# element36-io/hyperfridge-r0

Hardware: NVIDIA B200
Metric: po2=20 segments/sec (synthetic rv32im-shaped segment, W=256); camt53 proof seconds measured on a 37-segment proof (camt53.proof_seconds) (higher is better)
Workload: dtype u32 (BabyBear mod p, Montgomery)

## Files before the change

### hyperfridge-r0_b200/csrc/hfb200.cu

```cuda
#include "../../include/hfb200.h"
#include "prover.cuh"
#include "probe.cuh"
#include "verify.cuh"
#include <algorithm>
#include <atomic>
#include <condition_variable>
#include <deque>
#include <map>
#include <memory>
#include <thread>

using namespace hf;

struct hfb200_ctx {
    Prover p;
    std::vector<uint32_t> seal;
#ifndef HFB200_EMU
    cudaEvent_t marks[4] = {nullptr, nullptr, nullptr, nullptr};
#endif
};

static const char kOomMessage[] = "hfb200: out of memory while reporting an error";
static const char* dup_err(const std::string& s) {
    char* m = (char*)std::malloc(s.size() + 1);
// ... 417 lines not shown
            }
            hfb200_segment_job& j = jobs[idx];
            const auto t0 = std::chrono::steady_clock::now();
            j.attempts++;
            const char* err = nullptr;
            int injected = -1;
            {
                std::lock_guard<std::mutex> lock(pool->inject_mu);
                auto it = pool->inject.find(w);
                if (it != pool->inject.end()) { if (it->second.first == 0) { injected = it->second.second; pool->inject.erase(it); } else it->second.first--; }
            }
            if (injected == 0) err = dup_err("CUDA error cudaErrorLaunchFailure (injected by hfb200_pool_inject_fault)");
            else if (injected == 1) err = dup_err("injected non-device failure");
            if (!err && !j.code) {
                const auto it = pool->control.find(j.po2);
                if (it == pool->control.end()) err = dup_err("code is NULL and no control group was loaded for this po2 (hfb200_pool_load_control)");
                else if (!(sl.ctx->p.control_cached && sl.ctx->p.po2 == j.po2 && sl.ctx->p.control_gen == it->second.gen)) {
                    uint32_t root[8];
                    err = control_root_impl(sl.ctx, j.po2, it->second.code, root, it->second.gen);
                }
            }
            if (!err && pool->accum_fn) err = prove_job_with_accum(pool, sl.ctx, j, idx);
            else if (!err) err = hfb200_prove_segment(sl.ctx, j.po2, j.globals, j.code, j.data, j.blind_seed, j.seal_out, j.seal_cap, &j.seal_words);
            j.device = sl.device;
            j.ms = std::chrono::duration<float, std::milli>(std::chrono::steady_clock::now() - t0).count();
            bool requeue = false, retire = false;
            if (err && is_device_fault(err)) {
                pool->drop_ctx(sl);
                try { sl.ctx = pool->make_ctx(sl.device); } catch (...) { sl.ctx = nullptr; retire = true; }
                requeue = j.attempts < HFB200_POOL_MAX_ATTEMPTS;
            }
            {
                std::lock_guard<std::mutex> lock(mu);
                if (err && is_device_fault(err)) { pool->total_faults++; sl.faults++; if (!retire) pool->contexts_recreated++; }
                if (requeue) { hfb200_free_error(err); err = nullptr; pool->total_retries++; pending.push_back(idx); }
                j.error = err;
                if (retire) sl.retired = true;
                inflight--;
            }
            cv.notify_all();
            if (retire) {
                std::lock_guard<std::mutex> lock(mu);
                size_t spare = pool->slots.size();
                for (size_t k = 0; k < pool->slots.size(); k++) if (!taken[k] && !pool->slots[k].retired && pool->slots[k].ctx) { spare = k; break; }
                if (spare == pool->slots.size()) return;
                taken[spare] = 1;
                w = spare;
            }
        }
    };
    std::vector<std::thread> th;
    std::map<int, size_t> started;
    for (size_t w = 0; w < pool->slots.size(); w++) {
        const auto& sl = pool->slots[w];
        if (sl.retired || !sl.ctx) continue;
        if (started[sl.device] >= per_device_cap[sl.device]) continue;
        started[sl.device]++;
        taken[w] = 1;
        th.emplace_back(worker, w);
    }
    for (auto& t : th) t.join();
    for (size_t idx : pending) if (!jobs[idx].error) jobs[idx].error = dup_err("no healthy context left in the pool (every worker retired after CUDA errors)");
    for (size_t i = 0; i < n_jobs; i++)
        if (jobs[i].error) return dup_err(std::string("job ") + std::to_string(i) + ": " + jobs[i].error);
    API_CATCH
}

const char* hfb200_pool_load_control(hfb200_pool* pool, uint32_t po2, const uint32_t* code) {
    API_TRY
    if (!pool) throw Err("hfb200_pool_load_control: NULL pool");
    if (code) pool->control[po2] = hfb200_pool::Control{code, pool->next_gen++}; else pool->control.erase(po2);
    API_CATCH
}

const char* hfb200_pool_set_accum(hfb200_pool* pool, hfb200_accum_fn fn, void* user) {
    API_TRY
    if (!pool) throw Err("hfb200_pool_set_accum: NULL pool");
    pool->accum_fn = fn;
    pool->accum_user = fn ? user : nullptr;
    API_CATCH
}

void hfb200_pool_destroy(hfb200_pool* pool) { delete pool; }

struct DevBuf {
    Dev& d; uint32_t* p;
    DevBuf(Dev& dev, size_t words) : d(dev), p((uint32_t*)dev.alloc(words * 4)) {}
    ~DevBuf() { d.free(p); }
};

const char* hfb200_op_interpolate_ntt(hfb200_ctx* ctx, uint32_t* io, size_t count, size_t n, int zk_shift) {
    API_TRY
    if (!ctx || !io) throw Err("op_interpolate_ntt: NULL argument");
    ctx->p.bind();
    Dev& d = ctx->p.dev;
    const int lg = ilog2(n);
    if ((1ull << lg) != n || lg > 24 || count == 0) throw Err("op_interpolate_ntt: bad size");
    DevBuf b(d, count * n);
    d.h2d(b.p, io, count * n * 4);
    ctx->p.ntt.interpolate(b.p, n, b.p, n, (uint32_t)count, lg, zk_shift != 0);
    d.d2h(io, b.p, count * n * 4);
    d.sync();
    API_CATCH
}
const char* hfb200_op_expand_ntt(hfb200_ctx* ctx, uint32_t* out, const uint32_t* in, size_t count, size_t n_in, uint32_t expand_bits) {
    API_TRY
    if (!ctx || !out || !in) throw Err("op_expand_ntt: NULL argument");
    ctx->p.bind();
    Dev& d = ctx->p.dev;
    const int lg = ilog2(n_in);
    if ((1ull << lg) != n_in || lg + (int)expand_bits > 24 || (expand_bits != 0 && expand_bits != 2) || count == 0) throw Err("op_expand_ntt: bad size");
    DevBuf bi(d, count * n_in), bo(d, (count * n_in) << expand_bits);
    d.h2d(bi.p, in, count * n_in * 4);
    ctx->p.ntt.expand_evaluate(bi.p, n_in, bo.p, n_in << expand_bits, (uint32_t)count, lg, (int)expand_bits);
    d.d2h(out, bo.p, ((count * n_in) << expand_bits) * 4);
    d.sync();
    API_CATCH
}
const char* hfb200_op_lde(hfb200_ctx* ctx, uint32_t* out, const uint32_t* in, size_t count, size_t n_in) {
    API_TRY
    if (!ctx || !out || !in) throw Err("op_lde: NULL argument");
    ctx->p.bind();
    Dev& d = ctx->p.dev;
    const int lg = ilog2(n_in);
    if ((1ull << lg) != n_in || lg > 22 || count == 0) throw Err("op_lde: bad size");
    DevBuf bi(d, count * n_in), bs(d, count * n_in), bo(d, count * n_in * 4);
    d.h2d(bi.p, in, count * n_in * 4);
    ctx->p.ntt.lde(bi.p, n_in, bo.p, n_in * 4, bs.p, (uint32_t)count, lg);
    d.d2h(out, bo.p, count * n_in * 16);
    d.sync();
    API_CATCH
}
const char* hfb200_op_merkle(hfb200_ctx* ctx, const uint32_t* matrix, size_t rows, size_t cols, uint32_t* nodes_out) {
    API_TRY
    if (!ctx || !matrix || !nodes_out) throw Err("op_merkle: NULL argument");
    ctx->p.bind();
    Dev& d = ctx->p.dev;
    if ((1ull << ilog2(rows)) != rows || rows < 2 || cols == 0) throw Err("op_merkle: rows must be a power of two >= 2");
    DevBuf bm(d, rows * cols), bn(d, 2 * rows * 8);
    d.h2d(bm.p, matrix, rows * cols * 4);
    d.zero(bn.p, 8 * 4);
    ctx->p.merkle.build(bm.p, rows, (uint32_t)rows, (uint32_t)cols, bn.p);
    d.d2h(nodes_out, bn.p, 2 * rows * 8 * 4);
    d.sync();
    API_CATCH
}
const char* hfb200_op_poseidon2(hfb200_ctx* ctx, uint32_t* states, size_t n) {
    API_TRY
    if (!ctx || (!states && n)) throw Err("op_poseidon2: NULL argument");
    ctx->p.bind();
    Dev& d = ctx->p.dev;
    DevBuf b(d, n * 24);
    d.h2d(b.p, states, n * 24 * 4);
    d.launch<PermuteKernel, 128, 1>((unsigned)((n + 127) / 128), 1, 128, 0, b.p, (uint32_t)n);
    d.d2h(states, b.p, n * 24 * 4);
    d.sync();
    API_CATCH
}
const char* hfb200_op_fri_fold(hfb200_ctx* ctx, uint32_t* out, const uint32_t* in, size_t n, const uint32_t* mix4) {
    API_TRY
    if (!ctx || !out || !in || !mix4) throw Err("op_fri_fold: NULL argument");
    ctx->p.bind();
    Dev& d = ctx->p.dev;
    if (n < 16 || (n & 15)) throw Err("op_fri_fold: n must be a multiple of 16");
    DevBuf bi(d, 4 * n), bo(d, 4 * n / 16);
    d.h2d(bi.p, in, 4 * n * 4);
    FriFoldArgs fa{};
    fa.in = bi.p; fa.out = bo.p; fa.n = (uint32_t)n;
    const E4 fm = e4(mix4[0], mix4[1], mix4[2], mix4[3]);
    { E4 cur = e4_one(); for (int i = 0; i < 16; i++) { fa.mixpow[i] = cur; cur = e4_mul(cur, fm); } }
    d.launch<FriFoldKernel, 256, 1>((unsigned)((n / 16 + 255) / 256), 1, 256, 0, fa);
    d.d2h(out, bo.p, (4 * n / 16) * 4);
    d.sync();
    API_CATCH
}

const char* hfb200_bench_lde(hfb200_ctx* ctx, uint32_t po2, uint32_t count, uint32_t iters, float* ms_avg) {
    API_TRY
    if (!ctx || !ms_avg) throw Err("bench_lde: NULL argument");
    Prover& p = ctx->p;
    p.bind();
    p.layout(po2);
    if (count == 0 || count > p.cir.cd.w_data) throw Err("bench_lde: count must be in [1, w_data]");
    if (!p.have_trace) throw Err("bench_lde: call hfb200_witgen_synth first");
    const size_t N = (size_t)1 << po2;
    Timer t; t.init(p.dev.stream);
    p.ntt.lde(p.tr[GROUP_DATA], N, p.ev[GROUP_DATA], 4 * N, p.scratch, count, (int)po2);
    t.start();
    for (uint32_t i = 0; i < iters; i++) p.ntt.lde(p.tr[GROUP_DATA], N, p.ev[GROUP_DATA], 4 * N, p.scratch, count, (int)po2);
    t.stop();
    *ms_avg = t.ms() / (iters ? iters : 1);
    t.destroy();
    API_CATCH
}
const char* hfb200_bench_merkle(hfb200_ctx* ctx, uint32_t po2, uint32_t count, uint32_t iters, float* ms_avg) {
    API_TRY
    if (!ctx || !ms_avg) throw Err("bench_merkle: NULL argument");
    Prover& p = ctx->p;
    p.bind();
    p.layout(po2);
    if (count == 0 || count > p.cir.cd.w_data) throw Err("bench_merkle: count must be in [1, w_data]");
    const size_t D = (size_t)4 << po2;
    Timer t; t.init(p.dev.stream);
    p.merkle.build(p.ev[GROUP_DATA], D, (uint32_t)D, count, p.nodes[GROUP_DATA]);
    t.start();
    for (uint32_t i = 0; i < iters; i++) p.merkle.build(p.ev[GROUP_DATA], D, (uint32_t)D, count, p.nodes[GROUP_DATA]);
    t.stop();
    *ms_avg = t.ms() / (iters ? iters : 1);
    t.destroy();
    API_CATCH
}

const char* hfb200_verify_segment(const hfb200_circuit_desc* c, const hfb200_circuit_ir* ir, const uint32_t* seal, size_t seal_words,
                                  const uint32_t* code_root, uint32_t* po2_out) {
    API_TRY
    if ((c == nullptr) == (ir == nullptr)) throw Err("hfb200_verify_segment: pass exactly one of circuit / ir");
    if (!seal || !code_root) throw Err("hfb200_verify_segment: NULL seal or code_root");
    VCircuit vc;
    if (c) vc.init_builtin(c->w_code, c->w_data, c->w_accum);
    else vc.init_ir(ir->w_code, ir->w_data, ir->w_accum, ir->n_mix, reinterpret_cast<const IrTap*>(ir->taps), ir->n_taps,
                    reinterpret_cast<const IrStep*>(ir->steps), ir->n_steps, ir->ret, ir->info);
    verify_segment(vc, seal, seal_words, code_root, po2_out);
    API_CATCH
}
const char* hfb200_verify_segments(const hfb200_circuit_desc* c, const hfb200_circuit_ir* ir, const uint32_t* const* seals, const size_t* seal_words,
                                   size_t n, const uint32_t* code_roots, uint32_t* po2_out, unsigned threads, size_t* first_bad) {
    API_TRY
    if ((c == nullptr) == (ir == nullptr)) throw Err("hfb200_verify_segments: pass exactly one of circuit / ir");
    if (n && (!seals || !seal_words || !code_roots)) throw Err("hfb200_verify_segments: NULL argument");
    if (first_bad) *first_bad = n;
    VCircuit vc;
    if (c) vc.init_builtin(c->w_code, c->w_data, c->w_accum);
    else vc.init_ir(ir->w_code, ir->w_data, ir->w_accum, ir->n_mix, reinterpret_cast<const IrTap*>(ir->taps), ir->n_taps,
                    reinterpret_cast<const IrStep*>(ir->steps), ir->n_steps, ir->ret, ir->info);
    p2_host_consts();
    unsigned nt = threads ? threads : std::thread::hardware_concurrency();
    if (nt == 0) nt = 1;
    if (nt > n) nt = (unsigned)n;
    std::vector<std::string> errs(n);
    std::vector<char> bad(n, 0);
    std::atomic<size_t> next{0};
    auto work = [&]() {
        for (size_t i = next.fetch_add(1); i < n; i = next.fetch_add(1)) {
            try {
                if (!seals[i]) throw Err("NULL seal");
                uint32_t po2 = 0;
                verify_segment(vc, seals[i], seal_words[i], code_roots + 8 * i, &po2);
                if (po2_out) po2_out[i] = po2;
            } catch (const std::exception& e) { errs[i] = e.what(); bad[i] = 1; } catch (...) { errs[i] = "unknown error"; bad[i] = 1; }
        }
    };
    std::vector<std::thread> pool;
    for (unsigned t = 1; t < nt; t++) pool.emplace_back(work);
    work();
    for (auto& t : pool) t.join();
    for (size_t i = 0; i < n; i++) if (bad[i]) { if (first_bad) *first_bad = i; throw Err("segment " + std::to_string(i) + ": " + errs[i]); }
    API_CATCH
}
static Digest8 digest_bytes_impl(const uint8_t* bytes, size_t n) {
    if (n >= P) throw Err("hfb200_digest_bytes: input too long");
    std::vector<uint32_t> el;
    el.reserve(1 + (n + 2) / 3);
    el.push_back(to_mont((uint32_t)n));
    for (size_t i = 0; i < n; i += 3) {
        uint32_t v = bytes[i];
        if (i + 1 < n) v |= (uint32_t)bytes[i + 1] << 8;
        if (i + 2 < n) v |= (uint32_t)bytes[i + 2] << 16;
        el.push_back(to_mont(v));
    }
    return host_hash_elems(el.data(), el.size());
}
static Digest8 digest_pair_impl(const uint32_t* a, const uint32_t* b) {
    p2_host_consts();
    uint32_t st[24] = {0};
    for (int i = 0; i < 8; i++) { st[i] = a[i]; st[8 + i] = b[i]; }
    p2_mix(st);
    Digest8 d; for (int i = 0; i < 8; i++) d.w[i] = st[i];
    return d;
}
static void claim_check_words(const uint32_t* w, const char* what) {
    for (int i = 0; i < 8; i++) if (w[i] >= P) throw Err(std::string("claim: ") + what + " digest holds a non-canonical field element");
}
const char* hfb200_digest_bytes(const uint8_t* bytes, size_t n, uint32_t* out8) {
    API_TRY
    if ((!bytes && n) || !out8) throw Err("hfb200_digest_bytes: NULL argument");
    const Digest8 d = digest_bytes_impl(bytes, n);
    std::memcpy(out8, d.w, 32);
    API_CATCH
}
const char* hfb200_digest_pair(const uint32_t* a8, const uint32_t* b8, uint32_t* out8) {
    API_TRY
    if (!a8 || !b8 || !out8) throw Err("hfb200_digest_pair: NULL argument");
    claim_check_words(a8, "left"); claim_check_words(b8, "right");
    const Digest8 d = digest_pair_impl(a8, b8);
    std::memcpy(out8, d.w, 32);
    API_CATCH
}
const char* hfb200_claim_encode(const hfb200_claim* c, uint32_t* globals) {
    API_TRY
    if (!c || !globals) throw Err("hfb200_claim_encode: NULL argument");
    if (c->exit_code > 1) throw Err("hfb200_claim_encode: exit_code must be HFB200_EXIT_HALTED or HFB200_EXIT_SYSTEM_SPLIT");
    claim_check_words(c->pre, "pre"); claim_check_words(c->post, "post"); claim_check_words(c->output, "output");
    globals[1] = c->exit_code ? ONE : 0u;
    std::memcpy(globals + 8, c->pre, 32); std::memcpy(globals + 16, c->post, 32); std::memcpy(globals + 24, c->output, 32);
    API_CATCH
}
const char* hfb200_claim_decode(const uint32_t* seal, size_t seal_words, hfb200_claim* out) {
// ... 118 lines not shown
```

### hyperfridge-r0_b200/csrc/poseidon2.cuh

```cuda
#pragma once
#include "dev.cuh"

namespace hf {

#include "poseidon2_consts.inc"

struct P2Consts {
    uint32_t rc_first[96], rc_partial[21], rc_last[96], diag[24];
    uint32_t diag_std[24], diag_shoup[24];
};

static inline P2Consts p2_make_consts() {
    P2Consts c;
    for (int i = 0; i < 96; i++) { c.rc_first[i] = to_mont(P2_RC_FULL_FIRST[i]); c.rc_last[i] = to_mont(P2_RC_FULL_LAST[i]); }
    for (int i = 0; i < 21; i++) c.rc_partial[i] = to_mont(P2_RC_PARTIAL[i]);
    for (int i = 0; i < 24; i++) {
        c.diag[i] = to_mont(P2_M_INT_DIAG[i]);
        c.diag_std[i] = P2_M_INT_DIAG[i];
        c.diag_shoup[i] = (uint32_t)(((uint64_t)P2_M_INT_DIAG[i] << 32) / P);
    }
    return c;
}

#if !defined(HFB200_EMU)
__constant__ P2Consts g_p2c;
#define P2C_DEV g_p2c
#endif
static P2Consts g_p2c_host;
static inline const P2Consts& p2_host_consts() {
    static const bool once = (g_p2c_host = p2_make_consts(), true);
    (void)once;
    return g_p2c_host;
}

HD const P2Consts& p2c() {
#if defined(__CUDA_ARCH__)
    return P2C_DEV;
#else
    return g_p2c_host;
#endif
}

#ifndef P2_FADD_ALU
#define P2_FADD_ALU 0
#endif
HD uint32_t padd(uint32_t a, uint32_t b) {
#if defined(__CUDA_ARCH__) && P2_FADD_ALU
    const uint32_t x = __viaddmin_u32(a, b, 0xFFFFFFFFu);
    return __viaddmin_u32(x, 0u - P, x);
#else
    return fadd(a, b);
#endif
}
HD uint32_t fmul_lazy(uint32_t a, uint32_t b) {
    uint64_t o = (uint64_t)a * b;
    uint32_t m = (uint32_t)o * P_INV;
#ifdef __CUDA_ARCH__
    uint32_t mp = __umulhi(m, P);
#else
    uint32_t mp = (uint32_t)(((uint64_t)m * P) >> 32);
#endif
    return (uint32_t)(o >> 32) - mp + P;
}
HD uint32_t sbox7(uint32_t x) { uint32_t x2 = fmul(x, x), x3 = fmul(x2, x), x4 = fmul_lazy(x2, x2); return fmul(x3, x4); }
HD int32_t smul(int32_t a, int32_t b) {
    const int64_t o = (int64_t)a * b;
    const int32_t m = (int32_t)((uint32_t)o * P_INV);
#ifdef __CUDA_ARCH__
    const int32_t mp = __mulhi(m, (int32_t)P);
#else
    const int32_t mp = (int32_t)(((int64_t)m * (int64_t)P) >> 32);
#endif
    return (int32_t)(o >> 32) - mp;
}
#ifndef P2_SIGNED_SBOX
#define P2_SIGNED_SBOX 1
#endif
HD uint32_t sbox7_rc(uint32_t s, uint32_t rc) {
#if P2_SIGNED_SBOX
    const int32_t x = (int32_t)(s + rc - P);
    const int32_t x2 = smul(x, x), x3 = smul(x2, x), x4 = smul(x2, x2);
    const uint32_t r = (uint32_t)smul(x3, x4);
    return umin32(r, r + P);
#else
    return sbox7(padd(s, rc));
#endif
}
HD uint32_t fmul_const(uint32_t x, uint32_t d, uint32_t dp) {
#ifdef __CUDA_ARCH__
    const uint32_t q = __umulhi(x, dp);
#else
    const uint32_t q = (uint32_t)(((uint64_t)x * dp) >> 32);
#endif
    const uint32_t r = x * d - q * P;
    return umin32(r, r - P);
}

#ifndef P2_DEFERRED_SUM
#define P2_DEFERRED_SUM 1
#endif
HD void p2_m_ext(uint32_t* s) {
#pragma unroll
    for (int c = 0; c < 24; c += 4) {
        uint32_t a = s[c], b = s[c + 1], cc = s[c + 2], d = s[c + 3];
        uint32_t t0 = padd(a, b), t1 = padd(cc, d);
        uint32_t t2 = padd(padd(b, b), t1), t3 = padd(padd(d, d), t0);
        uint32_t t4 = padd(t1, t1); t4 = padd(padd(t4, t4), t3);
        uint32_t t5 = padd(t0, t0); t5 = padd(padd(t5, t5), t2);
        s[c] = padd(t3, t5); s[c + 1] = t5; s[c + 2] = padd(t2, t4); s[c + 3] = t4;
    }
    uint32_t sum[4];
#pragma unroll
    for (int j = 0; j < 4; j++) sum[j] = padd(padd(padd(s[j], s[4 + j]), padd(s[8 + j], s[12 + j])), padd(s[16 + j], s[20 + j]));
#pragma unroll
    for (int i = 0; i < 24; i++) s[i] = padd(s[i], sum[i & 3]);
}

HD void p2_m_int(uint32_t* s, const P2Consts& k) {
    uint32_t sum = 0;
#pragma unroll
    for (int i = 0; i < 24; i++) sum = padd(sum, s[i]);
#pragma unroll
    for (int i = 0; i < 24; i++) s[i] = padd(sum, fmul_const(s[i], k.diag_std[i], k.diag_shoup[i]));
}

HD void p2_mix(uint32_t* s) {
    const P2Consts& k = p2c();
    p2_m_ext(s);
#pragma unroll 1
    for (int r = 0; r < 4; r++) {
#pragma unroll
        for (int i = 0; i < 24; i++) s[i] = sbox7_rc(s[i], k.rc_first[r * 24 + i]);
        p2_m_ext(s);
    }
#if P2_DEFERRED_SUM
    {
        uint32_t U = s[1];
#pragma unroll
        for (int i = 2; i < 24; i++) U = padd(U, s[i]);
#pragma unroll 1
        for (int r = 0; r < 21; r++) {
            s[0] = sbox7_rc(s[0], k.rc_partial[r]);
            const uint32_t S = padd(s[0], U);
            uint32_t t[24];
#pragma unroll
            for (int i = 0; i < 24; i++) t[i] = fmul_const(s[i], k.diag_std[i], k.diag_shoup[i]);
            uint32_t T = t[1];
#pragma unroll
            for (int i = 2; i < 24; i++) T = padd(T, t[i]);
#if P2_DEFERRED_SUM == 2
            uint32_t S2 = padd(S, S), S4 = padd(S2, S2), S8 = padd(S4, S4), S16 = padd(S8, S8);
            const uint32_t S23 = fsub(padd(S16, S8), S);
#else
            const uint32_t S23 = fmul_const(S, 23u, (uint32_t)((23ull << 32) / P));
#endif
            U = padd(T, S23);
            s[0] = padd(t[0], S);
#pragma unroll
            for (int i = 1; i < 24; i++) s[i] = fadd_lazy(t[i], S);
        }
#pragma unroll
        for (int i = 1; i < 24; i++) s[i] = umin32(s[i], s[i] - P);
    }
#else
#pragma unroll 1
    for (int r = 0; r < 21; r++) {
        s[0] = sbox7_rc(s[0], k.rc_partial[r]);
        p2_m_int(s, k);
    }
#endif
#pragma unroll 1
    for (int r = 0; r < 4; r++) {
#pragma unroll
        for (int i = 0; i < 24; i++) s[i] = sbox7_rc(s[i], k.rc_last[r * 24 + i]);
        p2_m_ext(s);
    }
}

struct HashRowsKernel {
    static constexpr bool kBarrier = false;
    HD static void run(const KCtx& cx, uint32_t*, const uint32_t* matrix, uint64_t col_stride, uint32_t rows, uint32_t cols, uint32_t* nodes) {
        const uint64_t r = (uint64_t)cx.bx * cx.nt + cx.tid;
        if (r >= rows) return;
        uint32_t s[24];
#pragma unroll
        for (int i = 0; i < 24; i++) s[i] = 0;
        const uint32_t* src = matrix + r;
        uint32_t c = 0;
        for (; c + 16 <= cols; c += 16) {
#pragma unroll
            for (int i = 0; i < 16; i++) s[i] = src[(uint64_t)(c + i) * col_stride];
            p2_mix(s);
        }
        if (c < cols || cols == 0) {
#pragma unroll
            for (int i = 0; i < 16; i++) s[i] = (c + i < cols) ? src[(uint64_t)(c + i) * col_stride] : 0u;
            p2_mix(s);
        }
        uint4* dst = reinterpret_cast<uint4*>(nodes + ((uint64_t)rows + r) * 8);
        dst[0] = make_uint4(s[0], s[1], s[2], s[3]);
        dst[1] = make_uint4(s[4], s[5], s[6], s[7]);
    }
};

struct HashFoldKernel {
    static constexpr bool kBarrier = false;
    HD static void run(const KCtx& cx, uint32_t*, uint32_t* nodes, uint32_t level_size) {
        const uint64_t t = (uint64_t)cx.bx * cx.nt + cx.tid;
        if (t >= level_size) return;
        const uint64_t i = level_size + t;
        const uint4* in = reinterpret_cast<const uint4*>(nodes + 2 * i * 8);
        uint32_t s[24];
        uint4 v0 = in[0], v1 = in[1], v2 = in[2], v3 = in[3];
        s[0] = v0.x; s[1] = v0.y; s[2] = v0.z; s[3] = v0.w; s[4] = v1.x; s[5] = v1.y; s[6] = v1.z; s[7] = v1.w;
        s[8] = v2.x; s[9] = v2.y; s[10] = v2.z; s[11] = v2.w; s[12] = v3.x; s[13] = v3.y; s[14] = v3.z; s[15] = v3.w;
#pragma unroll
        for (int k = 16; k < 24; k++) s[k] = 0;
        p2_mix(s);
        uint4* dst = reinterpret_cast<uint4*>(nodes + i * 8);
        dst[0] = make_uint4(s[0], s[1], s[2], s[3]);
        dst[1] = make_uint4(s[4], s[5], s[6], s[7]);
    }
};

struct HashFoldTailKernel {
    static constexpr bool kBarrier = true;
    HD static void run(const KCtx& cx, uint32_t*, uint32_t* nodes, uint32_t top) {
        for (uint32_t level = top; level >= 1; level >>= 1) {
            for (uint32_t t = cx.tid; t < level; t += cx.nt) {
                const uint64_t i = level + t;
                uint32_t s[24];
#pragma unroll
                for (int k = 0; k < 16; k++) s[k] = nodes[2 * i * 8 + k];
#pragma unroll
                for (int k = 16; k < 24; k++) s[k] = 0;
                p2_mix(s);
#pragma unroll
                for (int k = 0; k < 8; k++) nodes[i * 8 + k] = s[k];
            }
#ifdef __CUDA_ARCH__
            __threadfence_block();
#endif
            cx.sync();
        }
    }
};

#ifdef __CUDA_ARCH__
struct WarpConsts { uint32_t rcf[4], rcl[4], d, dp; };
__device__ __forceinline__ WarpConsts wp2_consts(int lane) {
    const P2Consts& k = p2c();
    WarpConsts w;
    const int l = lane < 24 ? lane : 0;
#pragma unroll
    for (int r = 0; r < 4; r++) { w.rcf[r] = lane < 24 ? k.rc_first[r * 24 + l] : 0u; w.rcl[r] = lane < 24 ? k.rc_last[r * 24 + l] : 0u; }
    w.d = k.diag_std[l]; w.dp = k.diag_shoup[l];
    return w;
}
__device__ __forceinline__ uint32_t wp2_m_ext(uint32_t x, int lane) {
    const int q = lane & ~3;
    const uint32_t a = __shfl_sync(0xffffffffu, x, q), b = __shfl_sync(0xffffffffu, x, q + 1);
    const uint32_t c = __shfl_sync(0xffffffffu, x, q + 2), d = __shfl_sync(0xffffffffu, x, q + 3);
    const uint32_t t0 = fadd(a, b), t1 = fadd(c, d);
    const uint32_t t2 = fadd(fadd(b, b), t1), t3 = fadd(fadd(d, d), t0);
    uint32_t t4 = fadd(t1, t1); t4 = fadd(fadd(t4, t4), t3);
    uint32_t t5 = fadd(t0, t0); t5 = fadd(fadd(t5, t5), t2);
    const int r = lane & 3;
    const uint32_t out = r == 0 ? fadd(t3, t5) : r == 1 ? t5 : r == 2 ? fadd(t2, t4) : t4;
    uint32_t s = out;
    s = fadd(s, __shfl_xor_sync(0xffffffffu, s, 4));
    s = fadd(s, __shfl_xor_sync(0xffffffffu, s, 8));
    s = fadd(s, __shfl_xor_sync(0xffffffffu, s, 16));
    return lane < 24 ? fadd(out, s) : 0u;
}
__device__ __forceinline__ uint32_t wp2_mix(uint32_t x, int lane, const WarpConsts& w) {
    const P2Consts& k = p2c();
    x = wp2_m_ext(x, lane);
#pragma unroll
    for (int r = 0; r < 4; r++) x = wp2_m_ext(sbox7_rc(x, w.rcf[r]), lane);
#pragma unroll 1
    for (int r = 0; r < 21; r++) {
        const uint32_t y = sbox7_rc(x, k.rc_partial[r]);
        if (lane == 0) x = y;
        uint32_t s = x;
#pragma unroll
        for (int off = 16; off >= 1; off >>= 1) s = fadd(s, __shfl_xor_sync(0xffffffffu, s, off));
        x = lane < 24 ? fadd(s, fmul_const(x, w.d, w.dp)) : 0u;
    }
#pragma unroll
    for (int r = 0; r < 4; r++) x = wp2_m_ext(sbox7_rc(x, w.rcl[r]), lane);
    return x;
}
__device__ __forceinline__ void wp2_hash_pair(uint32_t* nodes, uint64_t i, int lane, const WarpConsts& w) {
    uint32_t x = lane < 16 ? nodes[2 * i * 8 + lane] : 0u;
    x = wp2_mix(x, lane, w);
    if (lane < 8) nodes[i * 8 + lane] = x;
}
#endif
struct HashFoldWarpKernel {
    static constexpr bool kBarrier = true;
    HD static void run(const KCtx& cx, uint32_t*, uint32_t* nodes, uint32_t level_size) {
#ifdef __CUDA_ARCH__
        const int lane = cx.tid & 31;
        const uint64_t wid = ((uint64_t)cx.bx * cx.nt + cx.tid) >> 5;
        if (wid >= level_size) return;
        const WarpConsts w = wp2_consts(lane);
        wp2_hash_pair(nodes, (uint64_t)level_size + wid, lane, w);
#else
        (void)cx; (void)nodes; (void)level_size;
#endif
    }
};
struct HashFoldWarpTailKernel {
    static constexpr bool kBarrier = true;
    HD static void run(const KCtx& cx, uint32_t*, uint32_t* nodes, uint32_t top) {
#ifdef __CUDA_ARCH__
        const int lane = cx.tid & 31, warp = cx.tid >> 5, nwarps = cx.nt >> 5;
        const WarpConsts w = wp2_consts(lane);
        for (uint32_t level = top; level >= 1; level >>= 1) {
            for (uint32_t t = warp; t < level; t += nwarps) wp2_hash_pair(nodes, (uint64_t)level + t, lane, w);
            __threadfence_block();
            __syncthreads();
        }
#else
        (void)cx; (void)nodes; (void)top;
#endif
    }
};

struct PermuteKernel {
    static constexpr bool kBarrier = false;
    HD static void run(const KCtx& cx, uint32_t*, uint32_t* states, uint32_t n) {
        const uint64_t t = (uint64_t)cx.bx * cx.nt + cx.tid;
        if (t >= n) return;
        uint32_t s[24];
        for (int i = 0; i < 24; i++) s[i] = states[t * 24 + i];
        p2_mix(s);
        for (int i = 0; i < 24; i++) states[t * 24 + i] = s[i];
    }
};

struct Merkle {
    Dev* dev = nullptr;
    void init(Dev* d) {
        dev = d;
        p2_host_consts();
#if !defined(HFB200_EMU)
        CUDA_CHECK(cudaMemcpyToSymbol(g_p2c, &g_p2c_host, sizeof(P2Consts)));
#endif
    }
    void build(const uint32_t* matrix, uint64_t col_stride, uint32_t rows, uint32_t cols, uint32_t* nodes) {
        const int T = 128;
        dev->launch<HashRowsKernel, 128, 1>((rows + T - 1) / T, 1, T, 0, matrix, col_stride, rows, cols, nodes);
        uint32_t level = rows / 2;
#ifndef HFB200_EMU
        static const uint32_t warp_max = [] { const char* e = std::getenv("HFB200_FOLD_WARP_MAX"); const int v = e ? std::atoi(e) : 0; return v >= 64 ? (uint32_t)v : 4096u; }();
        for (; level > warp_max; level >>= 1) dev->launch<HashFoldKernel, 128, 1>((level + T - 1) / T, 1, T, 0, nodes, level);
        for (; level > 32; level >>= 1) dev->launch<HashFoldWarpKernel, 256, 1>((level * 32 + 255) / 256, 1, 256, 0, nodes, level);
        if (level >= 1) dev->launch<HashFoldWarpTailKernel, 1024, 1>(1, 1, 1024, 0, nodes, level);
#else
        for (; level >= 512; level >>= 1) dev->launch<HashFoldKernel, 128, 1>((level + T - 1) / T, 1, T, 0, nodes, level);
        if (level >= 1) dev->launch<HashFoldTailKernel, 256, 1>(1, 1, 256, 0, nodes, level);
#endif
    }
};

struct Digest8 { uint32_t w[8]; };

static inline Digest8 host_hash_elems(const uint32_t* in, size_t n) {
    p2_host_consts();
    uint32_t s[24] = {0};
    size_t used = 0; bool any = false;
    for (size_t i = 0; i < n; i++) {
        s[used++] = in[i];
        if (used == 16) { p2_mix(s); used = 0; any = true; }
    }
    if (used != 0 || !any) { for (size_t k = used; k < 16; k++) s[k] = 0; p2_mix(s); }
    Digest8 d; for (int i = 0; i < 8; i++) d.w[i] = s[i];
    return d;
}

struct HostRng {
    uint32_t cells[24] = {0};
    int pool_used = 0;
    void mix(const uint32_t* d8) {
        p2_host_consts();
        if (pool_used != 0) { p2_mix(cells); pool_used = 0; }
        for (int i = 0; i < 8; i++) cells[i] = fadd(cells[i], d8[i]);
        p2_mix(cells);
    }
    uint32_t random_elem() { if (pool_used == 16) { p2_mix(cells); pool_used = 0; } return cells[pool_used++]; }
    E4 random_ext() { uint32_t a = random_elem(), b = random_elem(), c = random_elem(), d = random_elem(); return e4(a, b, c, d); }
    uint32_t random_bits(unsigned bits) {
        uint32_t v = from_mont(random_elem());
        for (int i = 0; i < 3; i++) { uint32_t n = from_mont(random_elem()); if (v == 0) v = n; }
        return v & (uint32_t)((1ull << bits) - 1);
    }
};

static constexpr char PROOF_SYSTEM_INFO[17] = "RISC0_STARK:v1__";
static constexpr char BUILTIN_CIRCUIT_INFO[17] = "SYNTH_RV32IM:v1_";
static constexpr char DEFAULT_IR_CIRCUIT_INFO[17] = "RV32IM:v2_______";
static inline void set_circuit_info(char* dst, bool data_defined, const uint8_t* info16) {
    bool given = false;
    if (info16) for (int i = 0; i < 16; i++) given = given || info16[i] != 0;
    if (!data_defined) std::memcpy(dst, BUILTIN_CIRCUIT_INFO, 17);
    else if (given) { std::memcpy(dst, info16, 16); dst[16] = 0; }
    else std::memcpy(dst, DEFAULT_IR_CIRCUIT_INFO, 17);
}
static inline Digest8 protocol_info_digest(const char* info16) {
    uint32_t e[16];
    for (int i = 0; i < 16; i++) e[i] = to_mont((uint32_t)(uint8_t)info16[i]);
    return host_hash_elems(e, 16);
}
static inline Digest8 transcript_header(HostRng& rng, const char* circuit_info16, const uint32_t* globals, size_t n_globals, uint32_t po2) {
    rng.mix(protocol_info_digest(PROOF_SYSTEM_INFO).w);
    rng.mix(protocol_info_digest(circuit_info16).w);
    std::vector<uint32_t> header(globals, globals + n_globals);
    header.push_back(po2);
    const Digest8 d = host_hash_elems(header.data(), header.size());
    rng.mix(d.w);
    return d;
}

}
```

Measured before the change: 20.04.

## Run Poseidon2 partial rounds as int8 tensor-core GEMMs via tcgen05

New measurement: 22.07 (median of 6 runs). 1.1x the previous value.

```diff
diff --git a/hyperfridge-r0_b200/csrc/hfb200.cu b/hyperfridge-r0_b200/csrc/hfb200.cu
--- a/hyperfridge-r0_b200/csrc/hfb200.cu
+++ b/hyperfridge-r0_b200/csrc/hfb200.cu
@@ -593,7 +593,7 @@
     Dev& d = ctx->p.dev;
     DevBuf b(d, n * 24);
     d.h2d(b.p, states, n * 24 * 4);
-    d.launch<PermuteKernel, 128, 1>((unsigned)((n + 127) / 128), 1, 128, 0, b.p, (uint32_t)n);
+    ctx->p.merkle.permute(b.p, (uint32_t)n);
     d.d2h(states, b.p, n * 24 * 4);
     d.sync();
     API_CATCH
diff --git a/hyperfridge-r0_b200/csrc/poseidon2.cuh b/hyperfridge-r0_b200/csrc/poseidon2.cuh
--- a/hyperfridge-r0_b200/csrc/poseidon2.cuh
+++ b/hyperfridge-r0_b200/csrc/poseidon2.cuh
@@ -8,7 +8,50 @@
 struct P2Consts {
     uint32_t rc_first[96], rc_partial[21], rc_last[96], diag[24];
     uint32_t diag_std[24], diag_shoup[24];
-};
+    int32_t tri_c[21];
+};
+
+static constexpr uint32_t P2TC_K1 = 96, P2TC_N1 = 80;
+static constexpr uint32_t P2TC_K2 = 192, P2TC_N2 = 96;
+static constexpr uint32_t P2TC_B1_BYTES = P2TC_K1 * P2TC_N1, P2TC_B_BYTES = P2TC_B1_BYTES + P2TC_K2 * P2TC_N2;
+HD uint32_t p2tc_off(uint32_t row, uint32_t k, uint32_t K) { return (row >> 3) * (K * 8) + (k >> 4) * 128 + (row & 7) * 16 + (k & 15); }
+struct P2TcTables {
+    uint8_t b[P2TC_B_BYTES];
+};
+
+static inline uint32_t p2_mod_mul(uint32_t a, uint32_t b) { return (uint32_t)((uint64_t)a * b % P); }
+static inline std::vector<std::vector<uint32_t>> p2_m_int_powers() {
+    std::vector<std::vector<uint32_t>> pw(22, std::vector<uint32_t>(24 * 24, 0));
+    for (int i = 0; i < 24; i++) pw[0][i * 24 + i] = 1;
+    for (int k = 1; k < 22; k++)
+        for (int o = 0; o < 24; o++)
+            for (int i = 0; i < 24; i++) {
+                uint64_t acc = p2_mod_mul(P2_M_INT_DIAG[o], pw[k - 1][o * 24 + i]);
+                for (int l = 0; l < 24; l++) acc += pw[k - 1][l * 24 + i];
+                pw[k][o * 24 + i] = (uint32_t)(acc % P);
+            }
+    return pw;
+}
+static inline void p2tc_put_output(uint8_t* b, uint32_t K, uint32_t o, const uint32_t* m, int n_in) {
+    for (int i = 0; i < n_in; i++)
+        for (uint32_t bb = 0; bb < 4; bb++) {
+            const uint32_t c = to_mont(p2_mod_mul(m[i], 1u << (8 * bb)));
+            for (uint32_t j = 0; j < 4; j++) b[p2tc_off(4 * o + j, 4 * i + bb, K)] = (uint8_t)(c >> (8 * j));
+        }
+}
+static inline P2TcTables p2_make_tc_tables() {
+    P2TcTables t;
+    std::memset(t.b, 0, sizeof t.b);
+    const auto pw = p2_m_int_powers();
+    uint32_t m[45];
+    for (uint32_t r = 1; r <= 20; r++) p2tc_put_output(t.b, P2TC_K1, r - 1, &pw[r][0], 24);
+    for (uint32_t o = 0; o < 24; o++) {
+        for (int i = 0; i < 24; i++) m[i] = pw[21][o * 24 + i];
+        for (int j = 0; j < 21; j++) m[24 + j] = pw[21 - j][o * 24];
+        p2tc_put_output(t.b + P2TC_B1_BYTES, P2TC_K2, o, m, 45);
+    }
+    return t;
+}
 
 static inline P2Consts p2_make_consts() {
     P2Consts c;
@@ -19,16 +62,24 @@
         c.diag_std[i] = P2_M_INT_DIAG[i];
         c.diag_shoup[i] = (uint32_t)(((uint64_t)P2_M_INT_DIAG[i] << 32) / P);
     }
+    const auto pw = p2_m_int_powers();
+    c.tri_c[0] = 0;
+    for (int k = 1; k < 21; k++) {
+        const uint32_t v = to_mont(pw[k][0]);
+        c.tri_c[k] = v > (P - 1) / 2 ? (int32_t)v - (int32_t)P : (int32_t)v;
+    }
     return c;
 }
 
 #if !defined(HFB200_EMU)
 __constant__ P2Consts g_p2c;
 #define P2C_DEV g_p2c
+__device__ __align__(16) uint8_t g_p2tc_b[P2TC_B_BYTES];
 #endif
 static P2Consts g_p2c_host;
+static P2TcTables g_p2tc_host;
 static inline const P2Consts& p2_host_consts() {
-    static const bool once = (g_p2c_host = p2_make_consts(), true);
+    static const bool once = (g_p2c_host = p2_make_consts(), g_p2tc_host = p2_make_tc_tables(), true);
     (void)once;
     return g_p2c_host;
 }
@@ -124,15 +175,19 @@
     for (int i = 0; i < 24; i++) s[i] = padd(sum, fmul_const(s[i], k.diag_std[i], k.diag_shoup[i]));
 }
 
+HD void p2_full_rounds(uint32_t* s, const uint32_t* rc) {
+#pragma unroll 1
+    for (int r = 0; r < 4; r++) {
+#pragma unroll
+        for (int i = 0; i < 24; i++) s[i] = sbox7_rc(s[i], rc[r * 24 + i]);
+        p2_m_ext(s);
+    }
+}
+
 HD void p2_mix(uint32_t* s) {
     const P2Consts& k = p2c();
     p2_m_ext(s);
-#pragma unroll 1
-    for (int r = 0; r < 4; r++) {
-#pragma unroll
-        for (int i = 0; i < 24; i++) s[i] = sbox7_rc(s[i], k.rc_first[r * 24 + i]);
-        p2_m_ext(s);
-    }
+    p2_full_rounds(s, k.rc_first);
 #if P2_DEFERRED_SUM
     {
         uint32_t U = s[1];
@@ -169,57 +224,278 @@
         p2_m_int(s, k);
     }
 #endif
-#pragma unroll 1
-    for (int r = 0; r < 4; r++) {
-#pragma unroll
-        for (int i = 0; i < 24; i++) s[i] = sbox7_rc(s[i], k.rc_last[r * 24 + i]);
-        p2_m_ext(s);
-    }
-}
+    p2_full_rounds(s, k.rc_last);
+}
+
+#ifndef P2_TC
+#define P2_TC 1
+#endif
+static constexpr uint32_t P2TC_A_BYTES = 128 * P2TC_K2;
+static constexpr size_t P2TC_SMEM = P2TC_A_BYTES + P2TC_B_BYTES + 32;
+static constexpr uint32_t P2TC_TMEM_COLS = 128;
+
+struct P2Tc {
+#ifdef __CUDA_ARCH__
+    uint8_t* a;
+    uint8_t* b;
+    uint64_t* bar;
+    uint32_t* tslot;
+    uint32_t tmem, phase, row;
+    bool b_wait;
+#else
+    uint32_t w[48];
+#endif
+};
+
+#ifdef __CUDA_ARCH__
+__device__ __forceinline__ void tc_fence_before() { asm volatile("tcgen05.fence::before_thread_sync;" ::: "memory"); }
+__device__ __forceinline__ void tc_fence_after() { asm volatile("tcgen05.fence::after_thread_sync;" ::: "memory"); }
+__device__ __forceinline__ uint64_t p2tc_desc(uint32_t saddr, uint32_t K) {
+    return (uint64_t)((saddr & 0x3FFFFu) >> 4) | ((uint64_t)(128u >> 4) << 16) | ((uint64_t)((8u * K) >> 4) << 32) | (1ull << 46);
+}
+#endif
+
+HD void p2tc_begin(P2Tc& tc, const KCtx& cx, uint32_t* smem) {
+#ifdef __CUDA_ARCH__
+    uint8_t* base = reinterpret_cast<uint8_t*>(smem);
+    tc.a = base;
+    tc.b = base + P2TC_A_BYTES;
+    tc.bar = reinterpret_cast<uint64_t*>(base + P2TC_A_BYTES + P2TC_B_BYTES);
+    tc.tslot = reinterpret_cast<uint32_t*>(tc.bar + 2);
+    tc.phase = 0;
+    tc.row = (uint32_t)cx.tid;
+    tc.b_wait = cx.tid == 0;
+    if (cx.tid == 0) {
+        mbar_init(&tc.bar[0], 1);
+        mbar_init(&tc.bar[1], 1);
+        mbar_init_fence();
+        mbar_expect_tx(&tc.bar[0], P2TC_B_BYTES);
+        tma_bulk_g2s(tc.b, g_p2tc_b, P2TC_B_BYTES, &tc.bar[0]);
+    }
+    if (cx.tid < 32) {
+        asm volatile("tcgen05.alloc.cta_group::1.sync.aligned.shared::cta.b32 [%0], %1;" ::"r"(smem_u32(tc.tslot)), "r"(P2TC_TMEM_COLS) : "memory");
+        asm volatile("tcgen05.relinquish_alloc_permit.cta_group::1.sync.aligned;" ::: "memory");
+    }
+    tc_fence_before();
+    __syncthreads();
+    tc_fence_after();
+    tc.tmem = *tc.tslot;
+#else
+    (void)tc; (void)cx; (void)smem;
+#endif
+}
+HD void p2tc_end(P2Tc& tc, const KCtx& cx) {
+#ifdef __CUDA_ARCH__
+    tc_fence_before();
+    __syncthreads();
+    if (cx.tid < 32) {
+        tc_fence_after();
+        asm volatile("tcgen05.dealloc.cta_group::1.sync.aligned.b32 %0, %1;" ::"r"(tc.tmem), "r"(P2TC_TMEM_COLS) : "memory");
+    }
+#else
+    (void)tc; (void)cx;
+#endif
+}
+HD void p2tc_put(P2Tc& tc, uint32_t w0, const uint32_t* v, uint32_t n) {
+#ifdef __CUDA_ARCH__
+#pragma unroll
+    for (uint32_t c = 0; c < n; c++)
+        *reinterpret_cast<uint4*>(tc.a + p2tc_off(tc.row, 4 * (w0 + 4 * c), P2TC_K2)) = make_uint4(v[4 * c], v[4 * c + 1], v[4 * c + 2], v[4 * c + 3]);
+#else
+    for (uint32_t i = 0; i < 4 * n; i++) tc.w[w0 + i] = v[i];
+#endif
+}
+HD void p2tc_gemm(P2Tc& tc, int g) {
+#ifdef __CUDA_ARCH__
+    asm volatile("fence.proxy.async.shared::cta;" ::: "memory");
+    tc_fence_before();
+    __syncthreads();
+    if (tc.row == 0) {
+        tc_fence_after();
+        if (tc.b_wait) { mbar_wait(&tc.bar[0], 0); tc.b_wait = false; }
+        const uint32_t K = g == 1 ? P2TC_K1 : P2TC_K2, N = g == 1 ? P2TC_N1 : P2TC_N2;
+        const uint32_t idesc = (2u << 4) | ((N >> 3) << 17) | ((128u >> 4) << 24);
+        const uint32_t a0 = smem_u32(tc.a), b0 = smem_u32(tc.b) + (g == 1 ? 0u : P2TC_B1_BYTES);
+        for (uint32_t kk = 0; kk < K / 32; kk++) {
+            const uint64_t ad = p2tc_desc(a0 + kk * 256, P2TC_K2), bd = p2tc_desc(b0 + kk * 256, K);
+            asm volatile("{\n.reg .pred p;\nsetp.ne.b32 p, %4, 0;\ntcgen05.mma.cta_group::1.kind::i8 [%0], %1, %2, %3, p;\n}\n"
+                         ::"r"(tc.tmem), "l"(ad), "l"(bd), "r"(idesc), "r"(kk) : "memory");
+        }
+        asm volatile("tcgen05.commit.cta_group::1.mbarrier::arrive::one.shared::cluster.b64 [%0];" ::"r"(smem_u32(&tc.bar[1])) : "memory");
+    }
+    mbar_wait(&tc.bar[1], tc.phase);
+    tc.phase ^= 1;
+    tc_fence_after();
+#else
+    (void)tc; (void)g;
+#endif
+}
+HD void p2tc_cols16(P2Tc& tc, int g, uint32_t c0, uint32_t* q) {
+#ifdef __CUDA_ARCH__
+    (void)g;
+    const uint32_t addr = tc.tmem + ((tc.row & ~31u) << 16) + c0;
+    asm volatile("tcgen05.ld.sync.aligned.32x32b.x16.b32 {%0, %1, %2, %3, %4, %5, %6, %7, %8, %9, %10, %11, %12, %13, %14, %15}, [%16];\n"
+                 "tcgen05.wait::ld.sync.aligned;\n"
+                 : "=r"(q[0]), "=r"(q[1]), "=r"(q[2]), "=r"(q[3]), "=r"(q[4]), "=r"(q[5]), "=r"(q[6]), "=r"(q[7]),
+                   "=r"(q[8]), "=r"(q[9]), "=r"(q[10]), "=r"(q[11]), "=r"(q[12]), "=r"(q[13]), "=r"(q[14]), "=r"(q[15])
+                 : "r"(addr) : "memory");
+#else
+    const uint8_t* a = reinterpret_cast<const uint8_t*>(tc.w);
+    const uint32_t K = g == 1 ? P2TC_K1 : P2TC_K2;
+    const uint8_t* b = g_p2tc_host.b + (g == 1 ? 0u : P2TC_B1_BYTES);
+    for (uint32_t n = 0; n < 16; n++) {
+        uint32_t acc = 0;
+        for (uint32_t k = 0; k < K; k++) acc += (uint32_t)a[k] * b[p2tc_off(c0 + n, k, K)];
+        q[n] = acc;
+    }
+#endif
+}
+HD uint32_t p2tc_reduce(const uint32_t* q) {
+    const uint32_t a = q[1] + (q[0] >> 8), b = q[2] + (a >> 8), c = q[3] + (b >> 8);
+    const uint32_t lo = q[0] + (q[1] << 8) + (q[2] << 16) + (q[3] << 24), hi = c >> 8;
+    const uint32_t m = lo * P_INV;
+#ifdef __CUDA_ARCH__
+    const uint32_t mp = __umulhi(m, P);
+#else
+    const uint32_t mp = (uint32_t)(((uint64_t)m * P) >> 32);
+#endif
+    const uint32_t r = hi - mp;
+    return umin32(r, r + P);
+}
+HD uint32_t p2tc_dot4(const int32_t* c, const int32_t* d, int n) {
+    int64_t v = 0;
+#pragma unroll
+    for (int j = 0; j < n; j++) v += (int64_t)c[j] * d[j];
+    const int32_t m = (int32_t)((uint32_t)v * P_INV);
+#ifdef __CUDA_ARCH__
+    const int32_t mp = __mulhi(m, (int32_t)P);
+#else
+    const int32_t mp = (int32_t)(((int64_t)m * (int64_t)P) >> 32);
+#endif
+    const uint32_t r = (uint32_t)((int32_t)(v >> 32) - mp);
+    return umin32(r, r + P);
+}
+
+HD void p2_mix_tc(uint32_t* s, P2Tc& tc) {
+    const P2Consts& k = p2c();
+    p2_m_ext(s);
+    p2_full_rounds(s, k.rc_first);
+    p2tc_put(tc, 0, s, 6);
+    p2tc_gemm(tc, 1);
+    uint32_t L[21];
+    L[0] = s[0];
+#pragma unroll
+    for (uint32_t c = 0; c < P2TC_N1; c += 16) {
+        uint32_t q[16];
+        p2tc_cols16(tc, 1, c, q);
+#pragma unroll
+        for (uint32_t o = 0; o < 4; o++) L[1 + c / 4 + o] = p2tc_reduce(q + 4 * o);
+    }
+    int32_t dlt[21];
+#pragma unroll
+    for (int r = 0; r < 21; r++) {
+        uint32_t y = L[r];
+#pragma unroll
+        for (int j0 = 0; j0 < r; j0 += 4) {
+            const int n = r - j0 < 4 ? r - j0 : 4;
+            int32_t cc[4], dd[4];
+#pragma unroll
+            for (int j = 0; j < 4; j++) if (j < n) { cc[j] = k.tri_c[r - j0 - j]; dd[j] = dlt[j0 + j]; }
+            y = fadd(y, p2tc_dot4(cc, dd, n));
+        }
+        const uint32_t d = fsub(sbox7_rc(y, k.rc_partial[r]), y);
+        dlt[r] = d > (P - 1) / 2 ? (int32_t)(d - P) : (int32_t)d;
+    }
+    uint32_t w[24];
+#pragma unroll
+    for (int j = 0; j < 21; j++) { const uint32_t u = (uint32_t)dlt[j]; w[j] = umin32(u, u + P); }
+    w[21] = w[22] = w[23] = 0;
+    p2tc_put(tc, 24, w, 6);
+    p2tc_gemm(tc, 2);
+#pragma unroll
+    for (uint32_t c = 0; c < P2TC_N2; c += 16) {
+        uint32_t q[16];
+        p2tc_cols16(tc, 2, c, q);
+#pragma unroll
+        for (uint32_t o = 0; o < 4; o++) s[c / 4 + o] = p2tc_reduce(q + 4 * o);
+    }
+    p2_full_rounds(s, k.rc_last);
+}
+
+struct P2Perm {
+#if P2_TC
+    static constexpr bool kAll = true;
+    static constexpr int kMinBlocks = 4;
+    static constexpr size_t kSmem = P2TC_SMEM;
+    P2Tc tc;
+    HD P2Perm(const KCtx& cx, uint32_t* smem) { p2tc_begin(tc, cx, smem); }
+    HD void mix(uint32_t* s) { p2_mix_tc(s, tc); }
+    HD void end(const KCtx& cx) { p2tc_end(tc, cx); }
+#else
+    static constexpr bool kAll = false;
+    static constexpr int kMinBlocks = 1;
+    static constexpr size_t kSmem = 0;
+    HD P2Perm(const KCtx&, uint32_t*) {}
+    HD void mix(uint32_t* s) { p2_mix(s); }
+    HD void end(const KCtx&) {}
+#endif
+};
 
 struct HashRowsKernel {
     static constexpr bool kBarrier = false;
-    HD static void run(const KCtx& cx, uint32_t*, const uint32_t* matrix, uint64_t col_stride, uint32_t rows, uint32_t cols, uint32_t* nodes) {
+    HD static void run(const KCtx& cx, uint32_t* smem, const uint32_t* matrix, uint64_t col_stride, uint32_t rows, uint32_t cols, uint32_t* nodes) {
         const uint64_t r = (uint64_t)cx.bx * cx.nt + cx.tid;
-        if (r >= rows) return;
+        const bool live = r < rows;
+        if (!live && !P2Perm::kAll) return;
+        P2Perm h(cx, smem);
         uint32_t s[24];
 #pragma unroll
         for (int i = 0; i < 24; i++) s[i] = 0;
-        const uint32_t* src = matrix + r;
+        const uint32_t* src = matrix + (live ? r : 0);
         uint32_t c = 0;
         for (; c + 16 <= cols; c += 16) {
 #pragma unroll
-            for (int i = 0; i < 16; i++) s[i] = src[(uint64_t)(c + i) * col_stride];
-            p2_mix(s);
+            for (int i = 0; i < 16; i++) s[i] = live ? src[(uint64_t)(c + i) * col_stride] : 0u;
+            h.mix(s);
         }
         if (c < cols || cols == 0) {
 #pragma unroll
-            for (int i = 0; i < 16; i++) s[i] = (c + i < cols) ? src[(uint64_t)(c + i) * col_stride] : 0u;
-            p2_mix(s);
-        }
-        uint4* dst = reinterpret_cast<uint4*>(nodes + ((uint64_t)rows + r) * 8);
-        dst[0] = make_uint4(s[0], s[1], s[2], s[3]);
-        dst[1] = make_uint4(s[4], s[5], s[6], s[7]);
+            for (int i = 0; i < 16; i++) s[i] = (live && c + i < cols) ? src[(uint64_t)(c + i) * col_stride] : 0u;
+            h.mix(s);
+        }
+        if (live) {
+            uint4* dst = reinterpret_cast<uint4*>(nodes + ((uint64_t)rows + r) * 8);
+            dst[0] = make_uint4(s[0], s[1], s[2], s[3]);
+            dst[1] = make_uint4(s[4], s[5], s[6], s[7]);
+        }
+        h.end(cx);
     }
 };
 
 struct HashFoldKernel {
     static constexpr bool kBarrier = false;
-    HD static void run(const KCtx& cx, uint32_t*, uint32_t* nodes, uint32_t level_size) {
+    HD static void run(const KCtx& cx, uint32_t* smem, uint32_t* nodes, uint32_t level_size) {
         const uint64_t t = (uint64_t)cx.bx * cx.nt + cx.tid;
-        if (t >= level_size) return;
-        const uint64_t i = level_size + t;
-        const uint4* in = reinterpret_cast<const uint4*>(nodes + 2 * i * 8);
+        const bool live = t < level_size;
+        if (!live && !P2Perm::kAll) return;
+        P2Perm h(cx, smem);
+        const uint64_t i = level_size + (live ? t : 0);
         uint32_t s[24];
-        uint4 v0 = in[0], v1 = in[1], v2 = in[2], v3 = in[3];
-        s[0] = v0.x; s[1] = v0.y; s[2] = v0.z; s[3] = v0.w; s[4] = v1.x; s[5] = v1.y; s[6] = v1.z; s[7] = v1.w;
-        s[8] = v2.x; s[9] = v2.y; s[10] = v2.z; s[11] = v2.w; s[12] = v3.x; s[13] = v3.y; s[14] = v3.z; s[15] = v3.w;
-#pragma unroll
-        for (int k = 16; k < 24; k++) s[k] = 0;
-        p2_mix(s);
-        uint4* dst = reinterpret_cast<uint4*>(nodes + i * 8);
-        dst[0] = make_uint4(s[0], s[1], s[2], s[3]);
-        dst[1] = make_uint4(s[4], s[5], s[6], s[7]);
+#pragma unroll
+        for (int k = 0; k < 24; k++) s[k] = 0;
+        if (live) {
+            const uint4* in = reinterpret_cast<const uint4*>(nodes + 2 * i * 8);
+            uint4 v0 = in[0], v1 = in[1], v2 = in[2], v3 = in[3];
+            s[0] = v0.x; s[1] = v0.y; s[2] = v0.z; s[3] = v0.w; s[4] = v1.x; s[5] = v1.y; s[6] = v1.z; s[7] = v1.w;
+            s[8] = v2.x; s[9] = v2.y; s[10] = v2.z; s[11] = v2.w; s[12] = v3.x; s[13] = v3.y; s[14] = v3.z; s[15] = v3.w;
+        }
+        h.mix(s);
+        if (live) {
+            uint4* dst = reinterpret_cast<uint4*>(nodes + i * 8);
+            dst[0] = make_uint4(s[0], s[1], s[2], s[3]);
+            dst[1] = make_uint4(s[4], s[5], s[6], s[7]);
+        }
+        h.end(cx);
     }
 };
 
@@ -330,13 +606,17 @@
 
 struct PermuteKernel {
     static constexpr bool kBarrier = false;
-    HD static void run(const KCtx& cx, uint32_t*, uint32_t* states, uint32_t n) {
+    HD static void run(const KCtx& cx, uint32_t* smem, uint32_t* states, uint32_t n) {
         const uint64_t t = (uint64_t)cx.bx * cx.nt + cx.tid;
-        if (t >= n) return;
+        const bool live = t < n;
+        if (!live && !P2Perm::kAll) return;
+        P2Perm h(cx, smem);
         uint32_t s[24];
-        for (int i = 0; i < 24; i++) s[i] = states[t * 24 + i];
-        p2_mix(s);
-        for (int i = 0; i < 24; i++) states[t * 24 + i] = s[i];
+        for (int i = 0; i < 24; i++) s[i] = live ? states[t * 24 + i] : 0u;
+        h.mix(s);
+        if (live)
+            for (int i = 0; i < 24; i++) states[t * 24 + i] = s[i];
+        h.end(cx);
     }
 };
 
@@ -347,19 +627,23 @@
         p2_host_consts();
 #if !defined(HFB200_EMU)
         CUDA_CHECK(cudaMemcpyToSymbol(g_p2c, &g_p2c_host, sizeof(P2Consts)));
-#endif
+        CUDA_CHECK(cudaMemcpyToSymbol(g_p2tc_b, g_p2tc_host.b, P2TC_B_BYTES));
+#endif
+    }
+    void permute(uint32_t* states, uint32_t n) {
+        dev->launch<PermuteKernel, 128, P2Perm::kMinBlocks>((n + 127) / 128, 1, 128, P2Perm::kSmem, states, n);
     }
     void build(const uint32_t* matrix, uint64_t col_stride, uint32_t rows, uint32_t cols, uint32_t* nodes) {
         const int T = 128;
-        dev->launch<HashRowsKernel, 128, 1>((rows + T - 1) / T, 1, T, 0, matrix, col_stride, rows, cols, nodes);
+        dev->launch<HashRowsKernel, 128, P2Perm::kMinBlocks>((rows + T - 1) / T, 1, T, P2Perm::kSmem, matrix, col_stride, rows, cols, nodes);
         uint32_t level = rows / 2;
 #ifndef HFB200_EMU
         static const uint32_t warp_max = [] { const char* e = std::getenv("HFB200_FOLD_WARP_MAX"); const int v = e ? std::atoi(e) : 0; return v >= 64 ? (uint32_t)v : 4096u; }();
-        for (; level > warp_max; level >>= 1) dev->launch<HashFoldKernel, 128, 1>((level + T - 1) / T, 1, T, 0, nodes, level);
+        for (; level > warp_max; level >>= 1) dev->launch<HashFoldKernel, 128, P2Perm::kMinBlocks>((level + T - 1) / T, 1, T, P2Perm::kSmem, nodes, level);
         for (; level > 32; level >>= 1) dev->launch<HashFoldWarpKernel, 256, 1>((level * 32 + 255) / 256, 1, 256, 0, nodes, level);
         if (level >= 1) dev->launch<HashFoldWarpTailKernel, 1024, 1>(1, 1, 1024, 0, nodes, level);
 #else
-        for (; level >= 512; level >>= 1) dev->launch<HashFoldKernel, 128, 1>((level + T - 1) / T, 1, T, 0, nodes, level);
+        for (; level >= 512; level >>= 1) dev->launch<HashFoldKernel, 128, P2Perm::kMinBlocks>((level + T - 1) / T, 1, T, P2Perm::kSmem, nodes, level);
         if (level >= 1) dev->launch<HashFoldTailKernel, 256, 1>(1, 1, 256, 0, nodes, level);
 #endif
     }
```
